# google/layered-scene-inference

Hardware: AMD Instinct MI355X
Metric: rendered views/sec (BxLxHxW splat+warp) (higher is better)
Workload: dtype f32; 1 GPU; cfg3: 4-layer LDI 256x768, batch 32 per GPU (32 total), trg_downsampling 0.5, kitti cameras, compose_layers, smooth disparities; launch=graph, input_sets_rotated=3, parallelism=batch-sharded replicas x1 (no collective)

## Files before the change

### layered-scene-inference_amd/csrc/lsi_splat_bwd_stream.hip

```cpp
#include <hip/hip_runtime.h>
#include <math.h>
#include <stdint.h>
#include <stdlib.h>

#include <type_traits>

#include "../../include/lsi_hip.h"
#include "lsi_common.h"
#include "lsi_splat_internal.h"

#pragma clang fp contract(off)

using namespace lsi;

namespace {

constexpr int BS_WPE = 2;
constexpr int BS_FENCE = 1;
constexpr int BS_T = 512;
constexpr int BS_NW = BS_T / 64;
constexpr int BS_SEG = 256;

struct BSCanvas {
  const float* img;
  const float* wts;
  const float* g_img;
  const float* g_wts;
};

struct BSArgs {
  const float* tex;
  const float* disp;
  const float* M;
  const float* mask;
  float* g_mask;
  int mask_sb, mask_sl, mask_sy;
  BSCanvas ci, cc;
  int vec4;
  float* g_tex;
  float* g_disp;
  int nt;
  int B, H, W, Ht, Wt, L, nseg;
  int tex_sb, tex_sl, tex_sy, disp_sb, disp_sl, disp_sy;
  float s, max_disp, zscale, zA, zB;
  int compose;
  int remap;
  int RS;
  int GR;
  float* gm_part;
  const float2* gd;
};

struct BSIn { float4 d4, t0, t1, t2, mk; };

__device__ __forceinline__ float4 bs_pre(float i0, float i1, float i2, float w,
                                         float g0, float g1, float g2, float gw) {
  const float inv = 1.0f / safe_den(w);
  return make_float4(g0 * inv, g1 * inv, g2 * inv,
                     gw - (g0 * i0 + g1 * i1 + g2 * i2) * inv);
}
__device__ __forceinline__ float4 bs_cell(const BSCanvas& c, size_t o) {
  return bs_pre(c.img[3 * o], c.img[3 * o + 1], c.img[3 * o + 2], c.wts[o],
                c.g_img[3 * o], c.g_img[3 * o + 1], c.g_img[3 * o + 2],
                c.g_wts ? c.g_wts[o] : 0.0f);
}
__device__ __forceinline__ float4 bs_G(const BSArgs& a, size_t oi, size_t oc) {
  float4 g = make_float4(0.f, 0.f, 0.f, 0.f);
  if (a.cc.g_img) g = bs_cell(a.cc, oc);
  if (a.ci.g_img) {
    const float4 h = bs_cell(a.ci, oi);
    g.x += h.x; g.y += h.y; g.z += h.z; g.w += h.w;
  }
  return g;
}
__device__ __forceinline__ void bs_cell4(const BSCanvas& c, size_t o, float4 (&g)[4],
                                         bool add) {
  const float4 ia = *reinterpret_cast<const float4*>(c.img + 3 * o);
  const float4 ib = *reinterpret_cast<const float4*>(c.img + 3 * o + 4);
  const float4 ic = *reinterpret_cast<const float4*>(c.img + 3 * o + 8);
  const float4 w = *reinterpret_cast<const float4*>(c.wts + o);
  const float4 ga = *reinterpret_cast<const float4*>(c.g_img + 3 * o);
  const float4 gb = *reinterpret_cast<const float4*>(c.g_img + 3 * o + 4);
  const float4 gc = *reinterpret_cast<const float4*>(c.g_img + 3 * o + 8);
  float4 gw = make_float4(0.f, 0.f, 0.f, 0.f);
  if (c.g_wts) gw = *reinterpret_cast<const float4*>(c.g_wts + o);
  float4 h[4];
  h[0] = bs_pre(ia.x, ia.y, ia.z, w.x, ga.x, ga.y, ga.z, gw.x);
  h[1] = bs_pre(ia.w, ib.x, ib.y, w.y, ga.w, gb.x, gb.y, gw.y);
  h[2] = bs_pre(ib.z, ib.w, ic.x, w.z, gb.z, gb.w, gc.x, gw.z);
  h[3] = bs_pre(ic.y, ic.z, ic.w, w.w, gc.y, gc.z, gc.w, gw.w);
#pragma unroll
  for (int k = 0; k < 4; ++k) {
    if (add) { g[k].x += h[k].x; g[k].y += h[k].y; g[k].z += h[k].z; g[k].w += h[k].w; }
    else g[k] = h[k];
  }
}

template <bool PACK>
__device__ __forceinline__ void bs_load(BSIn& o, const float* pd, const float* pt) {
  if (PACK) {
    o.d4 = *reinterpret_cast<const float4*>(pt);
    o.t0 = *reinterpret_cast<const float4*>(pt + 4);
    o.t1 = *reinterpret_cast<const float4*>(pt + 8);
    o.t2 = *reinterpret_cast<const float4*>(pt + 12);
  } else {
    o.d4 = *reinterpret_cast<const float4*>(pd);
    o.t0 = *reinterpret_cast<const float4*>(pt);
    o.t1 = *reinterpret_cast<const float4*>(pt + 4);
    o.t2 = *reinterpret_cast<const float4*>(pt + 8);
  }
}

typedef float __attribute__((ext_vector_type(4))) bs_f4v;
typedef const __attribute__((address_space(3))) bs_f4v bs_lds_f4;

template <bool IN_LDS, bool PACK, bool MASK, bool GRAD_M, bool WANT_DISP>
__device__ __forceinline__ void bs_run(const BSArgs& a, const float (&m)[8],
                                       BSIn (&set)[2], const float4* gt,
                                       size_t obi, size_t obc, int b,
                                       int l_lo, int NL, int ys, int nitem,
                                       int glo, int wave, int lane,
                                       float (&acc)[16]) {
  const int Wt = a.Wt, nseg = a.nseg;
  const int half = (Wt + 1) >> 1;
  const float s = a.s;
  const float xmax = (float)Wt - 1.0f, ymax = (float)a.Ht - 1.0f;
  const float inv_md = div_rn(1.0f, a.max_disp);
  const float zs_md = a.zscale * inv_md;
  const float* const g_tex_in = a.tex + (long)b * a.tex_sb + (long)l_lo * a.tex_sl;
  const float* const g_disp_in = a.disp + (long)b * a.disp_sb + (long)l_lo * a.disp_sl;
  const int px_last = a.W - 4;
  const float* const g_mask_in =
      MASK ? a.mask + (long)b * a.mask_sb + (long)l_lo * a.mask_sl : nullptr;
  float* const o_mask =
      MASK ? a.g_mask + ((size_t)l_lo * a.B + b) * ((size_t)a.H * a.W) + 4 * lane : nullptr;
  float* const o_tex = a.g_tex + ((size_t)l_lo * a.B + b) * ((size_t)a.H * a.W) * 3 + 12 * lane;
  float* const o_disp = a.g_disp + ((size_t)l_lo * a.B + b) * ((size_t)a.H * a.W) + 4 * lane;
  const size_t lay_px = (size_t)a.B * a.H * a.W;
  bs_lds_f4* const gt3 = (bs_lds_f4*)gt;

  struct Pos { int r, sg, l; };
  auto advance = [&](Pos& p, int n) {
    p.l += n;
    while (p.l >= NL) { p.l -= NL; ++p.sg; }
    while (p.sg >= nseg) { p.sg -= nseg; ++p.r; }
  };
  auto load_item = [&](BSIn& o, const Pos& p, bool live) {
    const Pos q = live ? p : Pos{0, 0, 0};
    const int px = min(q.sg * BS_SEG + 4 * lane, px_last);
    bs_load<PACK>(o, g_disp_in + (long)q.l * a.disp_sl + (long)(ys + q.r) * a.disp_sy + px,
                  g_tex_in + (long)q.l * a.tex_sl + (long)(ys + q.r) * a.tex_sy + (PACK ? 4 : 3) * px);
    if (MASK)
      o.mk = *reinterpret_cast<const float4*>(
          g_mask_in + (long)q.l * a.mask_sl + (long)(ys + q.r) * a.mask_sy + px);
  };
  auto item = [&](const BSIn& in, const Pos& p) {
    const int y = ys + p.r, sg = p.sg, l = p.l;
    const float py = (float)y + 0.5f;
    const float q1 = mrow(m, 1, 0.5f, py, 0.0f);
    const float Y = q1 * s - 0.5f;
    const Axis ay = splat_axis(Y, ymax);
    const bool yok = finite_f(Y);
    const int r0 = yok ? (int)ay.c0s : glo, r1 = yok ? (int)ay.c1s : glo;
    const float pym01 = py * m[1];
    const float dvn[4] = {in.d4.x, in.d4.y, in.d4.z, in.d4.w};
    const float dvp[4] = {in.d4.w, in.t0.w, in.t1.w, in.t2.w};
    const float txn[12] = {in.t0.x, in.t0.y, in.t0.z, in.t0.w, in.t1.x, in.t1.y,
                           in.t1.z, in.t1.w, in.t2.x, in.t2.y, in.t2.z, in.t2.w};
    const float txp[12] = {in.d4.x, in.d4.y, in.d4.z, in.t0.x, in.t0.y, in.t0.z,
                           in.t1.x, in.t1.y, in.t1.z, in.t2.x, in.t2.y, in.t2.z};
    const float (&dv)[4] = PACK ? dvp : dvn;
    const float (&tx)[12] = PACK ? txp : txn;
    const float mkv[4] = {in.mk.x, in.mk.y, in.mk.z, in.mk.w};
    float ot[12], od[4], om[4];
#pragma unroll
    for (int i = 0; i < 4; ++i) {
      const float d = dv[i];
      const float t0 = tx[3 * i], t1 = tx[3 * i + 1], t2 = tx[3 * i + 2];
      const float px = (float)(sg * BS_SEG + 4 * lane + i) + 0.5f;
      const float q0 = ((px * m[0] + pym01) + m[2]) + d * m[3];
      const float X = q0 * s - 0.5f;
      const bool ok = yok && finite_f(X) && finite_f(d);
      const Axis ax = splat_axis(X, xmax);
      float w0 = clamp_small(ax.w0 * ay.w0), w1 = clamp_small(ax.w1 * ay.w0);
      float w2 = clamp_small(ax.w0 * ay.w1), w3 = clamp_small(ax.w1 * ay.w1);
      if (!ok) { w0 = 0.f; w1 = 0.f; w2 = 0.f; w3 = 0.f; }
      const int c0 = ok ? (int)ax.c0s : 0, c1 = ok ? (int)ax.c1s : 0;
      float4 g0, g1, g2, g3;
      if (IN_LDS) {
        bs_lds_f4* ra = gt3 + (r0 - glo) * Wt;
        bs_lds_f4* rb = gt3 + (r1 - glo) * Wt;
        const int s0 = (c0 >> 1) + (c0 & 1) * half, s1 = (c1 >> 1) + (c1 & 1) * half;
        const bs_f4v v0 = ra[s0], v1 = ra[s1], v2 = rb[s0], v3 = rb[s1];
        g0 = make_float4(v0.x, v0.y, v0.z, v0.w); g1 = make_float4(v1.x, v1.y, v1.z, v1.w);
        g2 = make_float4(v2.x, v2.y, v2.z, v2.w); g3 = make_float4(v3.x, v3.y, v3.z, v3.w);
      } else {
        const size_t ra = (size_t)r0 * Wt, rb = (size_t)r1 * Wt;
        g0 = bs_G(a, obi + ra + c0, obc + ra + c0);
        g1 = bs_G(a, obi + ra + c1, obc + ra + c1);
        g2 = bs_G(a, obi + rb + c0, obc + rb + c0);
        g3 = bs_G(a, obi + rb + c1, obc + rb + c1);
      }
      float gsd = 0.0f;
      if (WANT_DISP) {
        const float2* gdl = a.gd + ((size_t)(l_lo + l) * a.B + b) * ((size_t)a.Ht * Wt);
        const size_t ra = (size_t)r0 * Wt, rb = (size_t)r1 * Wt;
        const float2 e0 = gdl[ra + c0], e1 = gdl[ra + c1];
        const float2 e2 = gdl[rb + c0], e3 = gdl[rb + c1];
        const float dz = ok ? d : 0.0f;
        g0.w = g0.w + (e0.y + dz * e0.x); g1.w = g1.w + (e1.y + dz * e1.x);
        g2.w = g2.w + (e2.y + dz * e2.x); g3.w = g3.w + (e3.y + dz * e3.x);
        gsd = __fmaf_rn(w3, e3.x, __fmaf_rn(w2, e2.x, __fmaf_rn(w1, e1.x, w0 * e0.x)));
      }
      const float xn = d * inv_md;
      const float ez = __builtin_amdgcn_exp2f(
          __fmaf_rn(__builtin_amdgcn_fmed3f(d, 0.0f, a.max_disp), a.zA, a.zB));
      const float zw = xn > 0.0f ? ez : 0.0f;
      const float S0 = __fmaf_rn(t0, g0.x, __fmaf_rn(t1, g0.y, __fmaf_rn(t2, g0.z, g0.w)));
      const float S1 = __fmaf_rn(t0, g1.x, __fmaf_rn(t1, g1.y, __fmaf_rn(t2, g1.z, g1.w)));
      const float S2 = __fmaf_rn(t0, g2.x, __fmaf_rn(t1, g2.y, __fmaf_rn(t2, g2.z, g2.w)));
      const float S3 = __fmaf_rn(t0, g3.x, __fmaf_rn(t1, g3.y, __fmaf_rn(t2, g3.z, g3.w)));
      const float a0 = __fmaf_rn(w3, g3.x, __fmaf_rn(w2, g2.x, __fmaf_rn(w1, g1.x, w0 * g0.x)));
      const float a1 = __fmaf_rn(w3, g3.y, __fmaf_rn(w2, g2.y, __fmaf_rn(w1, g1.y, w0 * g0.y)));
      const float a2 = __fmaf_rn(w3, g3.z, __fmaf_rn(w2, g2.z, __fmaf_rn(w1, g1.z, w0 * g0.z)));
      const float gpw = __fmaf_rn(w3, S3, __fmaf_rn(w2, S2, __fmaf_rn(w1, S1, w0 * S0)));
      const float pw = MASK ? zw * mkv[i] : zw;
      ot[3 * i] = a0 * pw; ot[3 * i + 1] = a1 * pw; ot[3 * i + 2] = a2 * pw;
      if (MASK) om[i] = gpw * zw;
      const float k0 = w0 != 0.0f ? pw * S0 : 0.0f, k1 = w1 != 0.0f ? pw * S1 : 0.0f;
      const float k2 = w2 != 0.0f ? pw * S2 : 0.0f, k3 = w3 != 0.0f ? pw * S3 : 0.0f;
      const float gX = -ax.v0 * (k0 * ay.w0 + k2 * ay.w1) + ax.v1 * (k1 * ay.w0 + k3 * ay.w1);
      const float inr = (xn >= 0.0f && xn <= 1.0f) ? 1.0f : 0.0f;
      float gD = gpw * pw * zs_md * inr;
      if (WANT_DISP) gD += gsd * pw;
      const float gd = (gX * s) * m[3] + gD;
      od[i] = ok ? gd : 0.0f;
      if (GRAD_M && ok && sg * BS_SEG + 4 * lane < a.W) {
        const float gY = -ay.v0 * (k0 * ax.w0 + k1 * ax.w1) +
                         ay.v1 * (k2 * ax.w0 + k3 * ax.w1);
        const float gq0 = gX * s, gq1 = gY * s;
        const float gn = -(gq0 * q0 + gq1 * q1 + gD * d);
        grad_m_add(acc, gq0, gq1, gn, gD, px, py, d);
      }
      if (((i + 1) & ((1 << BS_FENCE) - 1)) == 0 && i < 3) asm volatile("" ::: "memory");
    }
    const size_t po = (size_t)l * lay_px + (size_t)y * a.W + (size_t)sg * BS_SEG;
    if (sg * BS_SEG + 4 * lane < a.W) {
      float* pt = o_tex + 3 * po;
      if (a.nt) {
        store_stream_f4(pt, ot[0], ot[1], ot[2], ot[3]);
        store_stream_f4(pt + 4, ot[4], ot[5], ot[6], ot[7]);
        store_stream_f4(pt + 8, ot[8], ot[9], ot[10], ot[11]);
        store_stream_f4(o_disp + po, od[0], od[1], od[2], od[3]);
        if (MASK) store_stream_f4(o_mask + po, om[0], om[1], om[2], om[3]);
      } else {
        *reinterpret_cast<float4*>(pt) = make_float4(ot[0], ot[1], ot[2], ot[3]);
        *reinterpret_cast<float4*>(pt + 4) = make_float4(ot[4], ot[5], ot[6], ot[7]);
        *reinterpret_cast<float4*>(pt + 8) = make_float4(ot[8], ot[9], ot[10], ot[11]);
        *reinterpret_cast<float4*>(o_disp + po) = make_float4(od[0], od[1], od[2], od[3]);
        if (MASK)
          *reinterpret_cast<float4*>(o_mask + po) = make_float4(om[0], om[1], om[2], om[3]);
      }
    }
  };

  Pos p0{0, 0, 0}, p1{0, 0, 0};
  advance(p0, wave);
  advance(p1, wave + BS_NW);
  for (int it = wave; it < nitem; it += 2 * BS_NW) {
    item(set[0], p0);
    advance(p0, 2 * BS_NW);
    load_item(set[0], p0, it + 2 * BS_NW < nitem);
    if (it + BS_NW < nitem) item(set[1], p1);
    advance(p1, 2 * BS_NW);
    load_item(set[1], p1, it + 3 * BS_NW < nitem);
  }
}

template <bool PACK, bool MASK, bool GRAD_M, bool WANT_DISP>
__global__ __launch_bounds__(BS_T, BS_WPE) void splat_bwd_stream_kernel(BSArgs a) {
  extern __shared__ __attribute__((aligned(16))) unsigned char smem[];
  float4* const gt = reinterpret_cast<float4*>(smem);
  const int tid = threadIdx.x, lane = tid & 63;
  const int wave = __builtin_amdgcn_readfirstlane(tid >> 6);
  int bx = blockIdx.x, by = blockIdx.y, bz = blockIdx.z;
  if (a.remap) {
    const unsigned nbx = gridDim.x, L = gridDim.z;
    const unsigned lin = blockIdx.x + nbx * (blockIdx.y + gridDim.y * blockIdx.z);
    const unsigned xcd = lin & 7u, slot = lin >> 3;
    const unsigned l = slot % L, pair = (slot / L) * 8u + xcd;
    bz = (int)l;
    by = (int)(pair / nbx);
    bx = (int)(pair - (unsigned)by * nbx);
  }
  const int b = by;
  const int ys = bx * a.RS, ye = min(a.H, ys + a.RS);
  const int l_lo = a.compose ? 0 : bz;
  const int NL = a.compose ? a.L : 1;
  const int Wt = a.Wt;
  const int nseg = a.nseg;
  const int nitem = (ye - ys) * nseg * NL;

  BSIn set[2];
  {
    const float* const g_tex_in = a.tex + (long)b * a.tex_sb + (long)l_lo * a.tex_sl;
    const float* const g_disp_in = a.disp + (long)b * a.disp_sb + (long)l_lo * a.disp_sl;
#pragma unroll
    for (int k = 0; k < 2; ++k) {
      const int it = wave + k * BS_NW;
      const int itc = it < nitem ? it : 0;
      const int rs = itc / NL, l = itc - rs * NL;
      const int r = rs / nseg, sg = rs - r * nseg;
      const int px = min(sg * BS_SEG + 4 * lane, a.W - 4);
      bs_load<PACK>(set[k], g_disp_in + (long)l * a.disp_sl + (long)(ys + r) * a.disp_sy + px,
                    g_tex_in + (long)l * a.tex_sl + (long)(ys + r) * a.tex_sy + (PACK ? 4 : 3) * px);
      if (MASK)
        set[k].mk = *reinterpret_cast<const float4*>(
            a.mask + (long)b * a.mask_sb + (long)(l_lo + l) * a.mask_sl +
            (long)(ys + r) * a.mask_sy + px);
    }
  }

  const float* __restrict__ mg = a.M + 16 * b;
  float m[8];
#pragma unroll
  for (int k = 0; k < 8; ++k) m[k] = mg[k];
  const float s = a.s;
  const float ymax = (float)a.Ht - 1.0f;
  auto row_Y = [&](int y) {
    const float py = (float)y + 0.5f;
    return mrow(m, 1, 0.5f, py, 0.0f) * s - 0.5f;
  };
  int glo = 0, ghi = 0;
  {
    const Axis a0 = splat_axis(row_Y(ys), ymax), a1 = splat_axis(row_Y(max(ye - 1, ys)), ymax);
    const float lo = fminf(fminf(a0.c0s, a1.c0s), fminf(a0.c1s, a1.c1s));
    const float hi = fmaxf(fmaxf(a0.c0s, a1.c0s), fmaxf(a0.c1s, a1.c1s));
    glo = finite_f(lo) ? (int)lo : 0;
    ghi = finite_f(hi) ? (int)hi : 0;
  }
  const int grow = ghi - glo + 1;
  const bool in_lds = grow <= a.GR;
  const size_t P = (size_t)a.Ht * Wt;
  const size_t obi = ((size_t)l_lo * a.B + b) * P, obc = (size_t)b * P;
  if (in_lds) {
    const size_t c0 = (size_t)glo * Wt;
    const int n = grow * Wt;
    if (a.vec4) {
      const int half = (Wt + 1) >> 1;
      const float inv_wt = 1.0f / (float)Wt;
      for (int i = 4 * tid; i < n; i += 4 * BS_T) {
        float4 g[4];
#pragma unroll
        for (int k = 0; k < 4; ++k) g[k] = make_float4(0.f, 0.f, 0.f, 0.f);
        if (a.cc.g_img) bs_cell4(a.cc, obc + c0 + i, g, false);
        if (a.ci.g_img) bs_cell4(a.ci, obi + c0 + i, g, a.cc.g_img != nullptr);
        int row = (int)((float)i * inv_wt);
        int c = i - row * Wt;
        if (c >= Wt) { ++row; c -= Wt; }
        if (c < 0) { --row; c += Wt; }
        float4* dst = gt + row * Wt + (c >> 1);
        dst[0] = g[0]; dst[half] = g[1]; dst[1] = g[2]; dst[half + 1] = g[3];
      }
    } else {
      const int half = (Wt + 1) >> 1;
      for (int i = tid; i < n; i += BS_T) {
        const int row = i / Wt, c = i - row * Wt;
        gt[row * Wt + (c >> 1) + (c & 1) * half] = bs_G(a, obi + c0 + i, obc + c0 + i);
      }
    }
  }
  __syncthreads();
  float acc[16];
#pragma unroll
  for (int k = 0; k < 16; ++k) acc[k] = 0.0f;
  if (!GRAD_M && nitem <= 0) return;
  if (nitem > 0) {
    if (in_lds)
      bs_run<true, PACK, MASK, GRAD_M, WANT_DISP>(a, m, set, gt, obi, obc, b, l_lo, NL,
                                                  ys, nitem, glo, wave, lane, acc);
    else
      bs_run<false, PACK, MASK, GRAD_M, WANT_DISP>(a, m, set, gt, obi, obc, b, l_lo, NL,
                                                   ys, nitem, glo, wave, lane, acc);
  }
  if (GRAD_M) {
    __shared__ float red[BS_NW * 16];
    const size_t wg = ((size_t)b * gridDim.z + bz) * gridDim.x + bx;
    grad_m_block_sum<BS_NW>(acc, red, a.gm_part + 16 * wg);
  }
}

}

bool lsi_bwd_stream_applies(const LsiSplatDesc* d, const float* tex,
                            const float* disp, const float* mask,
                            const float* g_tex, const float* g_disp,
                            const float* g_mask) {
  if (const char* e = getenv("LSI_BWD_STREAM"))
    if (e[0] == '0') return false;
  if (d->path != LSI_PATH_STREAM || !(d->tune_window & LSI_STREAM_SIMPLE_BIT))
    return false;
  if (d->flags & LSI_WANT_DISP) return false;
  if (d->flags & LSI_HAS_MASK) {
    if (!mask || !g_mask || (d->flags & LSI_PACKED_RGBD) || d->mask_sx != 1) return false;
    const int64_t ms[] = {d->mask_sl, d->mask_sb, d->mask_sy};
    for (int64_t v : ms)
      if (v < 0 || v > 0x7fffffffLL || v % 4) return false;
    if (!aligned16(mask) || !aligned16(g_mask)) return false;
  }
  if (d->W % 4 != 0 || d->W < 4 || d->L < 1) return false;
  const bool pack = (d->flags & LSI_PACKED_RGBD) != 0;
  if (!pack && (d->tex_sc != 1 || d->tex_sx != 3 || d->disp_sx != 1)) return false;
  const int64_t st[] = {d->tex_sl, d->tex_sb, d->tex_sy, d->disp_sl, d->disp_sb, d->disp_sy};
  for (int64_t v : st)
    if (v < 0 || v > 0x7fffffffLL || v % 4) return false;
  if (!aligned16(tex) || (!pack && !aligned16(disp)) || !aligned16(g_tex) ||
      !aligned16(g_disp))
    return false;
  if ((long)d->B > 65535 || (long)d->L > 65535) return false;
  return true;
}

int lsi_bwd_stream_launch(const LsiSplatDesc* d, const float* tex,
                          const float* disp, const float* mask, const float* M,
                          const LsiBwdCanvas* ci, const LsiBwdCanvas* cc,
                          float* g_tex, float* g_disp, float* g_mask,
                          float* gm_part, int* gm_nper, hipStream_t stream,
                          const float2* gd) {
  BSArgs a;
  a.gm_part = gm_part;
  a.gd = gd;
  a.tex = tex; a.disp = disp; a.M = M; a.g_tex = g_tex; a.g_disp = g_disp;
  {
    static const char* nt_env = getenv("LSI_BWD_NT");
    a.nt = nt_env ? atoi(nt_env) : 0;
  }
  const bool has_mask = (d->flags & LSI_HAS_MASK) != 0;
  a.mask = has_mask ? mask : nullptr; a.g_mask = has_mask ? g_mask : nullptr;
  a.mask_sb = (int)d->mask_sb; a.mask_sl = (int)d->mask_sl; a.mask_sy = (int)d->mask_sy;
  const LsiBwdCanvas none = {nullptr, nullptr, nullptr, nullptr};
  const LsiBwdCanvas& i_ = ci ? *ci : none;
  const LsiBwdCanvas& c_ = cc ? *cc : none;
  a.ci = {i_.img, i_.wts, i_.g_img, i_.g_wts};
  a.cc = {c_.img, c_.wts, c_.g_img, c_.g_wts};
  a.vec4 = d->Wt % 4 == 0;
  for (const BSCanvas* c : {&a.ci, &a.cc})
    if (c->g_img)
      a.vec4 = a.vec4 && aligned16(c->img) && aligned16(c->wts) &&
               aligned16(c->g_img) && aligned16(c->g_wts);
  a.B = d->B; a.H = d->H; a.W = d->W; a.Ht = d->Ht; a.Wt = d->Wt; a.L = d->L;
  a.nseg = (d->W + BS_SEG - 1) / BS_SEG;
  a.tex_sb = (int)d->tex_sb; a.tex_sl = (int)d->tex_sl; a.tex_sy = (int)d->tex_sy;
  a.disp_sb = (int)d->disp_sb; a.disp_sl = (int)d->disp_sl; a.disp_sy = (int)d->disp_sy;
  a.s = d->trg_downsampling; a.max_disp = d->max_disp; a.zscale = d->zbuf_scale;
  const double l2e = 1.4426950408889634;
  a.zA = (float)((double)d->zbuf_scale * l2e / (double)d->max_disp);
  a.zB = (float)(-0.5 * (double)d->zbuf_scale * l2e);
  a.compose = (d->flags & LSI_COMPOSE) ? 1 : 0;
  auto rows_for = [&](int rs) { return (int)ceilf((float)rs * d->trg_downsampling) + 3; };
  auto bytes_for = [&](int rs) { return (size_t)rows_for(rs) * d->Wt * 16; };
  const size_t cap = 156 * 1024;
  int rs = 0;
  if (const char* e = getenv("LSI_BWD_STREAM_ROWS")) rs = atoi(e);
  if (rs <= 0) {
    rs = 8;
    for (int c : {32, 16, 8})
      if (bytes_for(c) <= cap) { rs = c; break; }
    const long nz = a.compose ? 1 : d->L;
    while (rs > 8 && (long)((d->H + rs - 1) / rs) * d->B * nz < 256) rs >>= 1;
  }
  a.RS = rs;
  a.GR = rows_for(rs);
  size_t lds = bytes_for(rs);
  if (lds > cap) { a.GR = 0; lds = 0; }
  const bool pack = (d->flags & LSI_PACKED_RGBD) != 0;
#define BS_FN(P_, M_, G_, D_) ((const void*)splat_bwd_stream_kernel<P_, M_, G_, D_>)
#define BS_PICK(G_, D_)                                                        \
  (pack ? BS_FN(true, false, G_, D_)                                            \
        : (has_mask ? BS_FN(false, true, G_, D_) : BS_FN(false, false, G_, D_)))
  const void* fn = gd ? (gm_part ? BS_PICK(true, true) : BS_PICK(false, true))
                      : (gm_part ? BS_PICK(true, false) : BS_PICK(false, false));
#undef BS_PICK
#undef BS_FN
  if (hipFuncSetAttribute(fn, hipFuncAttributeMaxDynamicSharedMemorySize,
                          (int)(lds > 0 ? lds : 16)) != hipSuccess) {
    (void)hipGetLastError();
    a.GR = 0; lds = 0;
    if (hipFuncSetAttribute(fn, hipFuncAttributeMaxDynamicSharedMemorySize, 16) !=
        hipSuccess)
      return LSI_ELAUNCH;
  }
  const dim3 grid((d->H + rs - 1) / rs, d->B, a.compose ? 1 : d->L);
  if (gm_nper) *gm_nper = (int)(grid.x * grid.z);
  {
    static const char* rm = getenv("LSI_BWD_REMAP");
    const long nwg = (long)grid.x * grid.y * grid.z;
    a.remap = (!a.compose && grid.z > 1 && nwg % (8L * grid.z) == 0 &&
               !(rm && rm[0] == '0')) ? 1 : 0;
  }
  void* kargs[1] = {&a};
  if (hipLaunchKernel(fn, grid, dim3(BS_T), kargs, lds, stream) != hipSuccess)
    return LSI_ELAUNCH;
  return hipGetLastError() == hipSuccess ? LSI_OK : LSI_ELAUNCH;
}
```

Baseline: 390,600 views/s.

## Stage gradient stores through per-wave LDS slab with nontemporal buffer stores

The texture-gradient output is now staged through a per-wave LDS slab and re-read, so each 128-bit store instruction writes one contiguous 1 KB span instead of three interleaved strided spans. All outputs use raw buffer stores with a nontemporal cache hint, and the buffer bounds replace the per-lane width branch. The input prefetch loop is restructured with empty asm register constraints that pin the loaded values, and the camera-matrix load is hoisted ahead of the first input loads. The cost is 24 KB of extra LDS per block, which counts against the row-tile budget and can lower occupancy. Nontemporal stores are now always on, where before they were off unless an environment variable enabled them.

```diff
diff --git a/layered-scene-inference_amd/csrc/lsi_splat_bwd_stream.hip b/layered-scene-inference_amd/csrc/lsi_splat_bwd_stream.hip
--- a/layered-scene-inference_amd/csrc/lsi_splat_bwd_stream.hip
+++ b/layered-scene-inference_amd/csrc/lsi_splat_bwd_stream.hip
@@ -39,7 +39,6 @@
   int vec4;
   float* g_tex;
   float* g_disp;
-  int nt;
   int B, H, W, Ht, Wt, L, nseg;
   int tex_sb, tex_sl, tex_sy, disp_sb, disp_sl, disp_sy;
   float s, max_disp, zscale, zA, zB;
@@ -47,11 +46,12 @@
   int remap;
   int RS;
   int GR;
+  int slab_off;
   float* gm_part;
   const float2* gd;
 };
 
-struct BSIn { float4 d4, t0, t1, t2, mk; };
+struct BSIn { lsi_v4f d4, t0, t1, t2, mk; };
 
 __device__ __forceinline__ float4 bs_pre(float i0, float i1, float i2, float w,
                                          float g0, float g1, float g2, float gw) {
@@ -99,24 +99,48 @@
 template <bool PACK>
 __device__ __forceinline__ void bs_load(BSIn& o, const float* pd, const float* pt) {
   if (PACK) {
-    o.d4 = *reinterpret_cast<const float4*>(pt);
-    o.t0 = *reinterpret_cast<const float4*>(pt + 4);
-    o.t1 = *reinterpret_cast<const float4*>(pt + 8);
-    o.t2 = *reinterpret_cast<const float4*>(pt + 12);
+    o.d4 = *reinterpret_cast<const lsi_v4f*>(pt);
+    o.t0 = *reinterpret_cast<const lsi_v4f*>(pt + 4);
+    o.t1 = *reinterpret_cast<const lsi_v4f*>(pt + 8);
+    o.t2 = *reinterpret_cast<const lsi_v4f*>(pt + 12);
   } else {
-    o.d4 = *reinterpret_cast<const float4*>(pd);
-    o.t0 = *reinterpret_cast<const float4*>(pt);
-    o.t1 = *reinterpret_cast<const float4*>(pt + 4);
-    o.t2 = *reinterpret_cast<const float4*>(pt + 8);
-  }
+    o.d4 = *reinterpret_cast<const lsi_v4f*>(pd);
+    o.t0 = *reinterpret_cast<const lsi_v4f*>(pt);
+    o.t1 = *reinterpret_cast<const lsi_v4f*>(pt + 4);
+    o.t2 = *reinterpret_cast<const lsi_v4f*>(pt + 8);
+  }
+}
+
+template <bool MASK>
+__device__ __forceinline__ void bs_use(BSIn& s) {
+  asm volatile("" : "+v"(s.d4), "+v"(s.t0), "+v"(s.t1), "+v"(s.t2));
+  if (MASK) asm volatile("" : "+v"(s.mk));
+}
+
+typedef __amdgpu_buffer_rsrc_t bs_rsrc;
+__device__ __forceinline__ bs_rsrc bs_out(float* p, int bytes) {
+  const uint64_t u = (uint64_t)p;
+  const uint64_t q = (uint64_t)(uint32_t)__builtin_amdgcn_readfirstlane((int)(uint32_t)u) |
+                     (uint64_t)(uint32_t)__builtin_amdgcn_readfirstlane((int)(u >> 32)) << 32;
+  return __builtin_amdgcn_make_buffer_rsrc((float*)q, 0, __builtin_amdgcn_readfirstlane(bytes),
+                                           0x00020000);
+}
+
+constexpr int BS_SLAB = BS_SEG * 12;
+__device__ __forceinline__ void bs_store_nt(bs_rsrc r, int off, lsi_v4f v) {
+  typedef unsigned __attribute__((ext_vector_type(4))) u4;
+  const u4 u = {__float_as_uint(v.x), __float_as_uint(v.y), __float_as_uint(v.z),
+                __float_as_uint(v.w)};
+  __builtin_amdgcn_raw_buffer_store_b128(u, r, off, 0, 2);
 }
 
 typedef float __attribute__((ext_vector_type(4))) bs_f4v;
+typedef __attribute__((address_space(3))) bs_f4v bs_lds_w4;
 typedef const __attribute__((address_space(3))) bs_f4v bs_lds_f4;
 
 template <bool IN_LDS, bool PACK, bool MASK, bool GRAD_M, bool WANT_DISP>
 __device__ __forceinline__ void bs_run(const BSArgs& a, const float (&m)[8],
-                                       BSIn (&set)[2], const float4* gt,
+                                       BSIn (&set)[2], const float4* gt, void* slab,
                                        size_t obi, size_t obc, int b,
                                        int l_lo, int NL, int ys, int nitem,
                                        int glo, int wave, int lane,
@@ -133,9 +157,9 @@
   const float* const g_mask_in =
       MASK ? a.mask + (long)b * a.mask_sb + (long)l_lo * a.mask_sl : nullptr;
   float* const o_mask =
-      MASK ? a.g_mask + ((size_t)l_lo * a.B + b) * ((size_t)a.H * a.W) + 4 * lane : nullptr;
-  float* const o_tex = a.g_tex + ((size_t)l_lo * a.B + b) * ((size_t)a.H * a.W) * 3 + 12 * lane;
-  float* const o_disp = a.g_disp + ((size_t)l_lo * a.B + b) * ((size_t)a.H * a.W) + 4 * lane;
+      MASK ? a.g_mask + ((size_t)l_lo * a.B + b) * ((size_t)a.H * a.W) : nullptr;
+  float* const o_tex = a.g_tex + ((size_t)l_lo * a.B + b) * ((size_t)a.H * a.W) * 3;
+  float* const o_disp = a.g_disp + ((size_t)l_lo * a.B + b) * ((size_t)a.H * a.W);
   const size_t lay_px = (size_t)a.B * a.H * a.W;
   bs_lds_f4* const gt3 = (bs_lds_f4*)gt;
 
@@ -151,7 +175,7 @@
     bs_load<PACK>(o, g_disp_in + (long)q.l * a.disp_sl + (long)(ys + q.r) * a.disp_sy + px,
                   g_tex_in + (long)q.l * a.tex_sl + (long)(ys + q.r) * a.tex_sy + (PACK ? 4 : 3) * px);
     if (MASK)
-      o.mk = *reinterpret_cast<const float4*>(
+      o.mk = *reinterpret_cast<const lsi_v4f*>(
           g_mask_in + (long)q.l * a.mask_sl + (long)(ys + q.r) * a.mask_sy + px);
   };
   auto item = [&](const BSIn& in, const Pos& p) {
@@ -245,35 +269,36 @@
       if (((i + 1) & ((1 << BS_FENCE) - 1)) == 0 && i < 3) asm volatile("" ::: "memory");
     }
     const size_t po = (size_t)l * lay_px + (size_t)y * a.W + (size_t)sg * BS_SEG;
-    if (sg * BS_SEG + 4 * lane < a.W) {
-      float* pt = o_tex + 3 * po;
-      if (a.nt) {
-        store_stream_f4(pt, ot[0], ot[1], ot[2], ot[3]);
-        store_stream_f4(pt + 4, ot[4], ot[5], ot[6], ot[7]);
-        store_stream_f4(pt + 8, ot[8], ot[9], ot[10], ot[11]);
-        store_stream_f4(o_disp + po, od[0], od[1], od[2], od[3]);
-        if (MASK) store_stream_f4(o_mask + po, om[0], om[1], om[2], om[3]);
-      } else {
-        *reinterpret_cast<float4*>(pt) = make_float4(ot[0], ot[1], ot[2], ot[3]);
-        *reinterpret_cast<float4*>(pt + 4) = make_float4(ot[4], ot[5], ot[6], ot[7]);
-        *reinterpret_cast<float4*>(pt + 8) = make_float4(ot[8], ot[9], ot[10], ot[11]);
-        *reinterpret_cast<float4*>(o_disp + po) = make_float4(od[0], od[1], od[2], od[3]);
-        if (MASK)
-          *reinterpret_cast<float4*>(o_mask + po) = make_float4(om[0], om[1], om[2], om[3]);
-      }
-    }
+    const int npx = min(BS_SEG, a.W - sg * BS_SEG);
+    const bs_rsrc bt = bs_out(o_tex + 3 * po, 12 * npx);
+    bs_lds_w4* const sl = (bs_lds_w4*)slab;
+    sl[3 * lane] = bs_f4v{ot[0], ot[1], ot[2], ot[3]};
+    sl[3 * lane + 1] = bs_f4v{ot[4], ot[5], ot[6], ot[7]};
+    sl[3 * lane + 2] = bs_f4v{ot[8], ot[9], ot[10], ot[11]};
+#pragma unroll
+    for (int n = 0; n < 3; ++n) bs_store_nt(bt, 1024 * n + 16 * lane, sl[64 * n + lane]);
+    bs_store_nt(bs_out(o_disp + po, 4 * npx), 16 * lane, lsi_v4f{od[0], od[1], od[2], od[3]});
+    if (MASK)
+      bs_store_nt(bs_out(o_mask + po, 4 * npx), 16 * lane, lsi_v4f{om[0], om[1], om[2], om[3]});
   };
-
+  auto step = [&](BSIn& s, Pos& p, bool more) {
+    bs_use<MASK>(s);
+    item(s, p);
+    advance(p, 2 * BS_NW);
+    load_item(s, p, more);
+  };
+
+  if (wave >= nitem) return;
   Pos p0{0, 0, 0}, p1{0, 0, 0};
   advance(p0, wave);
   advance(p1, wave + BS_NW);
-  for (int it = wave; it < nitem; it += 2 * BS_NW) {
-    item(set[0], p0);
-    advance(p0, 2 * BS_NW);
-    load_item(set[0], p0, it + 2 * BS_NW < nitem);
-    if (it + BS_NW < nitem) item(set[1], p1);
-    advance(p1, 2 * BS_NW);
-    load_item(set[1], p1, it + 3 * BS_NW < nitem);
+  bs_use<MASK>(set[0]);
+  bs_use<MASK>(set[1]);
+  for (int it = wave;;) {
+    step(set[0], p0, it + 2 * BS_NW < nitem);
+    if ((it += BS_NW) >= nitem) break;
+    step(set[1], p1, it + 2 * BS_NW < nitem);
+    if ((it += BS_NW) >= nitem) break;
   }
 }
 
@@ -283,6 +308,7 @@
   float4* const gt = reinterpret_cast<float4*>(smem);
   const int tid = threadIdx.x, lane = tid & 63;
   const int wave = __builtin_amdgcn_readfirstlane(tid >> 6);
+  void* const slab = smem + a.slab_off + wave * BS_SLAB;
   int bx = blockIdx.x, by = blockIdx.y, bz = blockIdx.z;
   if (a.remap) {
     const unsigned nbx = gridDim.x, L = gridDim.z;
@@ -301,6 +327,10 @@
   const int nseg = a.nseg;
   const int nitem = (ye - ys) * nseg * NL;
 
+  const float* __restrict__ mg = a.M + 16 * b;
+  float m[8];
+#pragma unroll
+  for (int k = 0; k < 8; ++k) m[k] = mg[k];
   BSIn set[2];
   {
     const float* const g_tex_in = a.tex + (long)b * a.tex_sb + (long)l_lo * a.tex_sl;
@@ -315,16 +345,12 @@
       bs_load<PACK>(set[k], g_disp_in + (long)l * a.disp_sl + (long)(ys + r) * a.disp_sy + px,
                     g_tex_in + (long)l * a.tex_sl + (long)(ys + r) * a.tex_sy + (PACK ? 4 : 3) * px);
       if (MASK)
-        set[k].mk = *reinterpret_cast<const float4*>(
+        set[k].mk = *reinterpret_cast<const lsi_v4f*>(
             a.mask + (long)b * a.mask_sb + (long)(l_lo + l) * a.mask_sl +
             (long)(ys + r) * a.mask_sy + px);
     }
   }
 
-  const float* __restrict__ mg = a.M + 16 * b;
-  float m[8];
-#pragma unroll
-  for (int k = 0; k < 8; ++k) m[k] = mg[k];
   const float s = a.s;
   const float ymax = (float)a.Ht - 1.0f;
   auto row_Y = [&](int y) {
@@ -377,10 +403,10 @@
   if (!GRAD_M && nitem <= 0) return;
   if (nitem > 0) {
     if (in_lds)
-      bs_run<true, PACK, MASK, GRAD_M, WANT_DISP>(a, m, set, gt, obi, obc, b, l_lo, NL,
+      bs_run<true, PACK, MASK, GRAD_M, WANT_DISP>(a, m, set, gt, slab, obi, obc, b, l_lo, NL,
                                                   ys, nitem, glo, wave, lane, acc);
     else
-      bs_run<false, PACK, MASK, GRAD_M, WANT_DISP>(a, m, set, gt, obi, obc, b, l_lo, NL,
+      bs_run<false, PACK, MASK, GRAD_M, WANT_DISP>(a, m, set, gt, slab, obi, obc, b, l_lo, NL,
                                                    ys, nitem, glo, wave, lane, acc);
   }
   if (GRAD_M) {
@@ -431,10 +457,6 @@
   a.gm_part = gm_part;
   a.gd = gd;
   a.tex = tex; a.disp = disp; a.M = M; a.g_tex = g_tex; a.g_disp = g_disp;
-  {
-    static const char* nt_env = getenv("LSI_BWD_NT");
-    a.nt = nt_env ? atoi(nt_env) : 0;
-  }
   const bool has_mask = (d->flags & LSI_HAS_MASK) != 0;
   a.mask = has_mask ? mask : nullptr; a.g_mask = has_mask ? g_mask : nullptr;
   a.mask_sb = (int)d->mask_sb; a.mask_sl = (int)d->mask_sl; a.mask_sy = (int)d->mask_sy;
@@ -460,19 +482,21 @@
   auto rows_for = [&](int rs) { return (int)ceilf((float)rs * d->trg_downsampling) + 3; };
   auto bytes_for = [&](int rs) { return (size_t)rows_for(rs) * d->Wt * 16; };
   const size_t cap = 156 * 1024;
+  const size_t slab = (size_t)BS_NW * BS_SLAB;
   int rs = 0;
   if (const char* e = getenv("LSI_BWD_STREAM_ROWS")) rs = atoi(e);
   if (rs <= 0) {
     rs = 8;
     for (int c : {32, 16, 8})
-      if (bytes_for(c) <= cap) { rs = c; break; }
+      if (bytes_for(c) + slab <= cap) { rs = c; break; }
     const long nz = a.compose ? 1 : d->L;
     while (rs > 8 && (long)((d->H + rs - 1) / rs) * d->B * nz < 256) rs >>= 1;
   }
   a.RS = rs;
   a.GR = rows_for(rs);
-  size_t lds = bytes_for(rs);
-  if (lds > cap) { a.GR = 0; lds = 0; }
+  size_t lds = bytes_for(rs) + slab;
+  if (lds > cap) { a.GR = 0; lds = slab; }
+  a.slab_off = (int)(lds - slab);
   const bool pack = (d->flags & LSI_PACKED_RGBD) != 0;
 #define BS_FN(P_, M_, G_, D_) ((const void*)splat_bwd_stream_kernel<P_, M_, G_, D_>)
 #define BS_PICK(G_, D_)                                                        \
@@ -485,9 +509,9 @@
   if (hipFuncSetAttribute(fn, hipFuncAttributeMaxDynamicSharedMemorySize,
                           (int)(lds > 0 ? lds : 16)) != hipSuccess) {
     (void)hipGetLastError();
-    a.GR = 0; lds = 0;
-    if (hipFuncSetAttribute(fn, hipFuncAttributeMaxDynamicSharedMemorySize, 16) !=
-        hipSuccess)
+    a.GR = 0; lds = slab; a.slab_off = 0;
+    if (hipFuncSetAttribute(fn, hipFuncAttributeMaxDynamicSharedMemorySize,
+                            (int)(lds > 0 ? lds : 16)) != hipSuccess)
       return LSI_ELAUNCH;
   }
   const dim3 grid((d->H + rs - 1) / rs, d->B, a.compose ? 1 : d->L);
```

Result: no change. 388,600 views/s (-0.5%).
